# vghuy17ck1/svt-av1-psyex

Measured on AMD Instinct MI355X. Metric: ME+RD-cost Mpixels/s (2160p10 preset-6), higher is better.
Workload: dtype u8 SAD / i32 transforms; 1 GPU; 3840x2160 10-bit synthetic pan sequence, preset 6 (M6) search controls at qp 35; step = 16 pictures (4 current pictures x ref distance 1,2,4,8; R=2): open-loop ME of all 2040 b64 + full-pel pred + RD chain (64x64,32x32,16x16 DCT_DCT, 10-bit, b quantizer; qcoeff + recon + scalars written); 3 picture sets alternate from step to step

## Files before the change

### include/svt_hip_dsp.h

```cpp
#ifndef SVT_HIP_DSP_H
#define SVT_HIP_DSP_H

#include <stdint.h>
#include "svt_hip_me.h"

#ifdef __cplusplus
extern "C" {
#endif

#define SVT_HIP_TX_SIZES_ALL 19
#define SVT_HIP_TX_TYPES 16

typedef struct SvtHipQuantRow {
    int16_t zbin[2], round[2], quant[2], quant_shift[2];
    int16_t round_fp[2], quant_fp[2];
    int16_t dequant[2];
} SvtHipQuantRow;

typedef struct SvtHipTxJob {
    uint32_t src_offset;
    uint32_t pred_offset;
    uint8_t  tx_type;
    uint8_t  quant_row;
    uint8_t  pf_shape;
// ... 27 lines not shown
typedef struct SvtHipFwdTxBatchDesc {
    uint8_t  tx_size, reserved[3];
    uint32_t n_jobs;
    uint32_t residual_stride;
    const int16_t     *residual;
    const SvtHipTxJob *jobs;
    int32_t           *coeff;
} SvtHipFwdTxBatchDesc;
int svt_hip_fwd_txfm_batch(SvtHipContext *ctx, const SvtHipFwdTxBatchDesc *d);

typedef struct SvtHipInvTxBatchDesc {
    uint8_t  bit_depth;
    uint8_t  sample_bytes;
    uint8_t  tx_size;
    uint8_t  reserved;
    uint32_t n_jobs;
    uint32_t pred_stride, recon_stride;
    const void        *pred;
    void              *recon;
    const SvtHipTxJob *jobs;
    const int32_t     *dqcoeff;
} SvtHipInvTxBatchDesc;
int svt_hip_inv_txfm_batch(SvtHipContext *ctx, const SvtHipInvTxBatchDesc *d);

typedef struct SvtHipBlockJob {
    uint32_t src_offset, ref_offset;
    uint8_t  width, height;
    uint8_t  subpel_x, subpel_y;
} SvtHipBlockJob;

typedef struct SvtHipBlockStatsDesc {
    uint8_t  bit_depth;
    uint8_t  temporal_layer_index;
    uint8_t  spy_rd;
    uint8_t  reserved;
    uint32_t n_jobs;
    uint32_t src_stride, ref_stride;
    const void           *src, *ref;
    const SvtHipBlockJob *jobs;
    uint32_t *sad;
    uint64_t *sse;
    uint32_t *variance;
    uint32_t *var_sse;
    uint32_t *satd;
    double    psy_rd;
    uint64_t *psy_energy;
// ... 157 lines not shown
```

### svt-av1-psyex_amd/api.py

```python
import ctypes as C
import os

import numpy as np

from . import abi

_HERE = os.path.dirname(os.path.abspath(__file__))
LIB_PATH = os.environ.get("SVT_HIP_LIBRARY") or os.path.join(_HERE, "libsvthip.so")
_lib = None

ERRORS = {1: "no usable gfx950 device", 2: "bad parameter", 3: "out of device memory", 4: "launch/stream error"}


class SvtHipError(RuntimeError):
    pass


def lib():
    global _lib
    if _lib is None:
        if not os.path.exists(LIB_PATH):
            raise SvtHipError(f"{LIB_PATH} is missing: build it with `make -C svt-av1-psyex_amd/csrc` "
                              "(or __graft_entry__.build()); there is no CPU fallback")
        try:
# ... 127 lines not shown
        self.check(lib().svt_hip_context_set_me_counting(self._h, 1 if on else 0), "svt_hip_context_set_me_counting")

    def me_dense_counters(self):
        v = (C.c_ulonglong * 2)()
        self.check(lib().svt_hip_me_dense_counters(self._h, v), "svt_hip_me_dense_counters")
        return int(v[0]), int(v[1])

    ME_DENSE_PATHS = ("fast", "partial_row", "skip_line", "short", "odd", "octet", "off")

    def set_me_dense_fast(self, on):
        self.check(lib().svt_hip_context_set_me_dense_fast(self._h, 1 if on else 0), "svt_hip_context_set_me_dense_fast")

    def set_me_dense_plan(self, plan):
        self.check(lib().svt_hip_context_set_me_dense_plan(self._h, int(plan)), "svt_hip_context_set_me_dense_plan")

    def me_dense_path_counters(self):
        n = len(self.ME_DENSE_PATHS)
        v = (C.c_ulonglong * (2 * n + 7))()
        self.check(lib().svt_hip_me_dense_path_counters(self._h, v), "svt_hip_me_dense_path_counters")
        out = {name: (int(v[2 * i]), int(v[2 * i + 1])) for i, name in enumerate(self.ME_DENSE_PATHS)}
        out["fast_rows"] = {8 * (m + 2): int(v[2 * n + m]) for m in range(7)}
        return out

    def me_dense_slots(self):
        L = lib()
        n = C.c_size_t()
        L.svt_hip_me_dense_slots.argtypes = [C.c_void_p, C.c_void_p, C.c_size_t, C.POINTER(C.c_size_t)]
        self.check(L.svt_hip_me_dense_slots(self._h, None, 0, C.byref(n)), "svt_hip_me_dense_slots")
        out = np.zeros(n.value // 16, dtype=[("key", "<u8"), ("org", "<u4"), ("size", "<u4")])
        self.check(L.svt_hip_me_dense_slots(self._h, out.ctypes.data_as(C.c_void_p), out.nbytes, C.byref(n)), "svt_hip_me_dense_slots")
        return out

    def upload(self, host_pyramid, device_pyramid=True):
        pic = C.c_void_p()
        full = host_pyramid.desc(2)
        if device_pyramid:
            rc = lib().svt_hip_pa_picture_create(self._h, C.byref(full), None, None, C.byref(pic))
        else:
            q, s = host_pyramid.desc(1), host_pyramid.desc(0)
            rc = lib().svt_hip_pa_picture_create(self._h, C.byref(full), C.byref(q), C.byref(s), C.byref(pic))
        self.check(rc, "svt_hip_pa_picture_create")
        return DevicePicture(self, pic, host_pyramid.picture_number)

    def upload_dev(self, dev_ptr, stride, width, height, pad, picture_number=0):
        pic = C.c_void_p()
        full = abi.PlaneDesc(dev_ptr, stride, pad, pad, width, height)
# ... 78 lines not shown
```

### svt-av1-psyex_amd/csrc/rd_kernel.hip

```cpp
#include <hip/hip_runtime.h>
#include <math.h>
#include <stdint.h>
#include <string.h>
#include <type_traits>
#include "svt_hip_internal.h"
#include "batch_host.h"
#include "../../include/svt_hip_dsp.h"

#include "txfm_core.h"

namespace {

struct RdParams {
    SvtHipRdBatchDesc d;
    const int16_t    *iscan[3];
    int               tx_size;
};

template <typename T> __device__ __forceinline__ int ldpix(const void *p, size_t i) { return (int)static_cast<const T *>(p)[i]; }

__host__ __device__ constexpr int rd_lanes_per_block(int ts) { return tx_wide(ts) > tx_high(ts) ? tx_wide(ts) : tx_high(ts); }
__host__ __device__ constexpr int rd_blocks_per_wave(int ts) { return 64 / rd_lanes_per_block(ts); }

#ifndef SVT_RD_WAVES_64
#define SVT_RD_WAVES_64 2
#endif
#ifndef SVT_RD_WAVES_32
#define SVT_RD_WAVES_32 4
#endif
#ifndef SVT_RD_RESIDUAL_AHEAD
#define SVT_RD_RESIDUAL_AHEAD 8
#endif
#ifndef SVT_RD_SCAN_AHEAD
#define SVT_RD_SCAN_AHEAD 16
#endif
#ifndef SVT_RD_WAVES_16
#define SVT_RD_WAVES_16 4
#endif
#ifndef SVT_RD_FOLD_INV_32LANE
#define SVT_RD_FOLD_INV_32LANE 1
#endif
__host__ __device__ constexpr int rd_bounded_btf(int ts) {
    return ((rd_lanes_per_block(ts) == 32 && tx_wide(ts) != tx_high(ts)) || (tx_wide(ts) == 64 && tx_high(ts) == 16)) ? 3 : 2;
}
#ifndef SVT_RD_CLAMP_FREE
#define SVT_RD_CLAMP_FREE 1
#endif
#ifndef SVT_RD_SKIP_ENTRY_CLAMPS
#define SVT_RD_SKIP_ENTRY_CLAMPS 1
#endif
#ifndef SVT_RD_PAIR_RESIDUAL_MAX
#define SVT_RD_PAIR_RESIDUAL_MAX 1
#endif
#ifndef SVT_RD_ROW_BOUND_FROM_QUANT
#define SVT_RD_ROW_BOUND_FROM_QUANT 1
#endif
__host__ __device__ constexpr bool rd_clamp_free_tier(int ts) {
    return tx_wide(ts) == tx_high(ts) && (SVT_RD_CLAMP_FREE == 1 ? tx_wide(ts) == 64 : SVT_RD_CLAMP_FREE == 2 && tx_wide(ts) >= 16);
}
__host__ __device__ constexpr bool rd_skip_entry_clamps(int ts) { return SVT_RD_SKIP_ENTRY_CLAMPS && rd_bounded_btf(ts) == 2; }
#ifdef SVT_RD_TIER_STATS
__device__ unsigned int g_rd_tier_stats[10];
#endif
template <bool FREE> __device__ __forceinline__ int ipass_tier(uint32_t wave_max_abs_input, int n, int clamp_bits) {
    if (FREE && ipass_clamp_free(wave_max_abs_input, n, clamp_bits)) return 2;
    return ipass_fits_18_bits(wave_max_abs_input, n) ? 1 : 0;
}
__host__ __device__ constexpr int rd_waves_per_simd(int ts) {
    return rd_lanes_per_block(ts) == 64 ? SVT_RD_WAVES_64 : rd_lanes_per_block(ts) == 32 ? SVT_RD_WAVES_32 : SVT_RD_WAVES_16;
}
template <int TS, int BD> __global__ void __launch_bounds__(64, rd_waves_per_simd(TS)) rd_tx_kernel(const RdParams p) {
    constexpr int W = tx_wide(TS), H = tx_high(TS), WP = W > 32 ? 32 : W, HP = H > 32 ? 32 : H, NP = WP * HP;
    constexpr int LW = rd_lanes_per_block(TS), BPW = rd_blocks_per_wave(TS);
    constexpr bool kShift32 = LW != 32;
    constexpr bool kFoldInv = LW != 32 || SVT_RD_FOLD_INV_32LANE;
    constexpr int kBtf = rd_bounded_btf(TS);
    constexpr bool kFree = rd_clamp_free_tier(TS), kSkipEntry = rd_skip_entry_clamps(TS);
    constexpr int PA = W + 1, PB = WP + 1;
    constexpr int ROW_CLAMP = BD == 8 ? 16 : 18, COL_CLAMP = 16;
    constexpr bool RECT = (W == 2 * H || H == 2 * W);
    using Pix = typename std::conditional<BD == 8, uint8_t, uint16_t>::type;
    __shared__ int32_t lds[BPW][H * PA];
    const int      lane = threadIdx.x, blk = lane / LW, l = lane % LW;
    const uint32_t job   = blockIdx.x * BPW + blk;
    const bool     valid = job < p.d.n_jobs;
    int32_t *A = lds[blk];
    const SvtHipTxJob jb = p.d.jobs[valid ? job : 0];
    const int tt = jb.tx_type & 15, vt = c_vtx[tt], ht = c_htx[tt];
    const bool ud = (vt == 2), lr = (ht == 2);
    const Pix *src  = static_cast<const Pix *>(p.d.src) + jb.src_offset;
    const Pix *pred = static_cast<const Pix *>(p.d.pred) + jb.pred_offset;
    const int8_t *fsh = c_fwd_shift[TS];
    const int bit_col = c_fwd_cos_col[ilog2c(W) - 2][ilog2c(H) - 2], bit_row = c_fwd_cos_row[ilog2c(W) - 2][ilog2c(H) - 2];

    constexpr int RUN = W < 8 ? W : 8, RPR = W / RUN;
    typedef Pix __attribute__((ext_vector_type(RUN), aligned(sizeof(Pix)))) RunU;
    uint32_t rmax = 0;
    {
        HiLo rhl;
        constexpr int NIT = (RPR * H + LW - 1) / LW, kResidualAhead = NIT < SVT_RD_RESIDUAL_AHEAD ? NIT : SVT_RD_RESIDUAL_AHEAD;
        for (int it0 = 0; it0 < NIT; it0 += kResidualAhead) {
            RunU sv[kResidualAhead], pv[kResidualAhead];
#pragma unroll
            for (int j = 0; j < kResidualAhead; j++) {
                const int i = l + (it0 + j) * LW;
                if (it0 + j < NIT && i < RPR * H) {
                    const int r = i / RPR, c = (i - r * RPR) * RUN;
                    sv[j] = *reinterpret_cast<const RunU *>(src + (size_t)r * p.d.src_stride + c);
                    pv[j] = *reinterpret_cast<const RunU *>(pred + (size_t)r * p.d.pred_stride + c);
                }
            }
#pragma unroll
// ... 2 lines not shown
                if (it0 + j < NIT && i < RPR * H) {
                    const int r = i / RPR, c = (i - r * RPR) * RUN;
                    static_assert(RUN % 2 == 0, "the extremes are taken per pair of samples");
#pragma unroll
                    for (int k = 0; k < RUN; k += 2) {
                        const int32_t d0 = (int16_t)((int16_t)sv[j][k] - (int16_t)pv[j][k]), d1 = (int16_t)((int16_t)sv[j][k + 1] - (int16_t)pv[j][k + 1]);
                        A[r * PA + c + k]     = d0;
                        A[r * PA + c + k + 1] = d1;
#if SVT_RD_PAIR_RESIDUAL_MAX
                        rhl.take(d0, d1);
#else
                        rhl.take(d0);
                        rhl.take(d1);
#endif
                    }
                }
            }
        }
        rmax = rhl.max_abs();
    }
    const bool fast_col = pass_fits_17_bits((uint32_t)__builtin_amdgcn_readfirstlane((int)wave_max(rmax)) << (fsh[0] > 0 ? fsh[0] : 0), H);
    __syncthreads();
    uint32_t cmax = 0;
    if (l < W) {
        int32_t x[H];
#pragma unroll
        for (int r = 0; r < H; r++) x[r] = A[(ud ? H - 1 - r : r) * PA + l];
        shift_vec<H>(x, fsh[0]);
        if constexpr (kBtf == 2) {
#pragma unroll
            for (int r = 0; r < H; r++) x[r] = held_in_vgpr(x[r]);
        }
        if (fast_col) fwd_1d_bounded<H, kShift32, kBtf>(x, vt, bit_col, fsh[1]); else { fwd_1d<H, 0>(x, vt, bit_col); shift_vec<H>(x, fsh[1]); }
        const int oc = lr ? W - 1 - l : l;
#pragma unroll
        for (int r = 0; r < H; r++) A[r * PA + oc] = x[r];
        cmax = vec_max_abs<H>(x);
    }
    const bool fast_row = pass_fits_17_bits((uint32_t)__builtin_amdgcn_readfirstlane((int)wave_max(cmax)), W);
    __syncthreads();
    uint32_t comax = 0;
    if (l < H) {
        int32_t x[W];
#pragma unroll
        for (int c = 0; c < W; c++) x[c] = A[l * PA + c];
        if (fast_row) fwd_1d_bounded<W, kShift32, kBtf>(x, ht, bit_row, fsh[2]); else { fwd_1d<W, 0>(x, ht, bit_row); shift_vec<W>(x, fsh[2]); }
        if constexpr (RECT) {
#pragma unroll
            for (int c = 0; c < W; c++) x[c] = rshift64((i64)x[c] * 5793, 12);
        }
#pragma unroll
        for (int c = 0; c < W; c++) A[l * PA + c] = x[c];
        comax = vec_max_abs<W>(x);
    }
    const uint32_t comax_w = (uint32_t)__builtin_amdgcn_readfirstlane((int)wave_max(comax));
    const bool q24 = comax_w < (1u << 16);
    __syncthreads();
    const int pf = jb.pf_shape & 3;
    const int keep_w = pf == 3 ? 1 : (W >> pf), keep_h = pf == 3 ? 1 : (H >> pf);
    u64 tq = 0;
    if (pf == 0) if constexpr (W > 32 || H > 32) {
        for (int i = l; i < W * H; i += LW) {
            const int r = i / W, c = i - r * W;
            if (r >= HP || c >= WP) { const int32_t v = A[r * PA + c]; tq += (u64)((i64)v * v); }
        }
// ... 6 lines not shown
    const uint8_t *qm = (tt < 9) ? p.d.qmatrix : nullptr, *iqm = (tt < 9) ? p.d.iqmatrix : nullptr;
    uint32_t satd = 0, eob = 0, qsum = 0;
    int32_t  dc_q = 0;
    u64      dres = 0, dpred = 0;
    int32_t *co_out = (p.d.coeff && valid) ? p.d.coeff + (size_t)job * NP : nullptr;
    int32_t *q_out  = (p.d.qcoeff && valid) ? p.d.qcoeff + (size_t)job * NP : nullptr;
    int32_t *dq_out = (p.d.dqcoeff && valid) ? p.d.dqcoeff + (size_t)job * NP : nullptr;
    const int32_t zb_c[2]  = {log_scale ? ((q.zbin[0] + (1 << (log_scale - 1))) >> log_scale) : q.zbin[0], log_scale ? ((q.zbin[1] + (1 << (log_scale - 1))) >> log_scale) : q.zbin[1]};
    const int32_t rnd_c[2] = {log_scale ? ((q.round[0] + (1 << (log_scale - 1))) >> log_scale) : q.round[0], log_scale ? ((q.round[1] + (1 << (log_scale - 1))) >> log_scale) : q.round[1]};
    const bool fast_q = q24 && !qm && p.d.quant_kind == 0 && !co_out && !dq_out && __all(pf == 0);
    constexpr int LS = tx_log_scale(TS), KT = LS == 2 ? 4 : 3;
    bool lane_lean = fast_q && q_out != nullptr && log_scale == LS;
    bool lane_row_free = false;
    {
        const int32_t  rndm = rnd_c[0] > rnd_c[1] ? rnd_c[0] : rnd_c[1], sm = q.quant_shift[0] > q.quant_shift[1] ? q.quant_shift[0] : q.quant_shift[1];
        const int32_t  dm = q.dequant[0] > q.dequant[1] ? q.dequant[0] : q.dequant[1], qm2 = (q.quant[0] > q.quant[1] ? q.quant[0] : q.quant[1]) + 65536;
        const bool     nonneg = (rnd_c[0] | rnd_c[1] | q.quant_shift[0] | q.quant_shift[1] | q.dequant[0] | q.dequant[1]) >= 0;
        uint32_t       tmax = comax_w + (uint32_t)(nonneg ? rndm : 0);
        if (BD == 8) tmax = tmax > 32767u ? 32767u : tmax;
        const u64 qvmax = ((((u64)tmax * (uint32_t)qm2) >> 11) * (u64)(uint32_t)(nonneg ? sm : 0)) >> (21 - LS);
        const u64 dqmax = (qvmax * (u64)(uint32_t)(nonneg ? dm : 0)) >> LS;
        const u64 M = dqmax > comax_w ? dqmax : (u64)comax_w;
        lane_lean = lane_lean && nonneg && tmax < (1u << (18 - KT)) && M < (1u << 16) && M * M * (NP / LW) < (1ull << 32);
        if constexpr (kFree && SVT_RD_ROW_BOUND_FROM_QUANT)
            lane_row_free = lane_lean && ipass_clamp_free((uint32_t)(RECT ? (M * 2896 + 2048) >> 12 : M), W, ROW_CLAMP);
    }
    const bool lean_q = __all(lane_lean);
    const bool row_free_q = kFree && SVT_RD_ROW_BOUND_FROM_QUANT && __all(lane_row_free);
    if (lean_q) {
        static_assert(NP % LW == 0, "every lane of a block walks the same number of coefficients");
        constexpr int kScanAhead = NP / LW < SVT_RD_SCAN_AHEAD ? ((NP / LW) & ~1) : SVT_RD_SCAN_AHEAD;
        static_assert(kScanAhead >= 2 && kScanAhead % 2 == 0 && NP / LW >= kScanAhead, "ahead of the loop");
        uint32_t scan2[kScanAhead / 2];
#pragma unroll
        for (int k = 0; k < kScanAhead; k += 2) scan2[k / 2] = (uint32_t)(uint16_t)iscan[l + LW * k] | ((uint32_t)(uint16_t)iscan[l + LW * (k + 1)] << 16);
        uint32_t dres32 = 0, dpred32 = 0;
        int32_t  last = -1;
        auto one = [&](int rc, int32_t zbr, int32_t rnd, uint32_t qq, uint32_t qshift, int32_t deq, int ahead = -1) {
            const int r = rc / WP, c = rc - r * WP;
            const int32_t co = A[r * PA + c], sg = (co >> 31) | 1, tu = __mul24(co, sg) + rnd;
            satd += (uint32_t)tu;
            uint32_t t = (uint32_t)tu;
            if (BD == 8) t = t > 32767u ? 32767u : t;
            const uint32_t tmp = umul24_lo(t, qq) >> 11;
            uint32_t qv = umul24_hi(tmp << KT, qshift);
            qv = tu >= zbr ? qv : 0u;
            const int32_t qs = __mul24((int32_t)qv, sg);
            int32_t dqs;
            if constexpr (LS == 0) dqs = __mul24(qs, deq);
            else dqs = __mul24(__mul24((int32_t)qv, deq) >> LS, sg);
            const int32_t dd = co - dqs;
// ... 146 lines not shown
        A[r * PB + c] = dqs;
        if (co_out) co_out[rc] = co;
        if (q_out) q_out[rc] = qs;
        if (dq_out) dq_out[rc] = dqs;
    }
    satd  = group_sum<LW>(satd);
    qsum  = group_sum<LW>(qsum);
    eob   = group_max<LW>(eob);
    dres  = group_sum<LW>(dres);
    dpred = group_sum<LW>(dpred);
    __syncthreads();
    int32_t xr[W];
    uint32_t irmax = 0;
    if (l < H) {
#pragma unroll
        for (int c = 0; c < W; c++) {
            int32_t v = (l < HP && c < WP) ? A[l * PB + c] : 0;
            if constexpr (RECT) v = rshift64((i64)v * 2896, 12);
            xr[c] = kSkipEntry ? v : clampv(v, BD + 8);
        }
        if (!row_free_q) irmax = vec_max_abs<W>(xr);
    }
    const uint32_t irmax_w = (uint32_t)__builtin_amdgcn_readfirstlane((int)wave_max(irmax));
    const int irow_tier = row_free_q ? 2 : ipass_tier<kFree>(irmax_w, W, ROW_CLAMP);
    uint32_t icmax = 0;
    if (l < H) {
        if (kSkipEntry && irmax_w >= (1u << (BD + 7))) {
#pragma unroll
            for (int c = 0; c < W; c++) xr[c] = clampv(xr[c], BD + 8);
        }
        if (irow_tier == 2) inv_1d_bounded<W, -1, kShift32, kFoldInv, kBtf>(xr, ht, c_inv_shift0[TS]);
        else if (irow_tier == 1) inv_1d_bounded<W, ROW_CLAMP, kShift32, kFoldInv, kBtf>(xr, ht, c_inv_shift0[TS]);
        else { inv_1d<W, ROW_CLAMP, 1>(xr, ht); shift_vec<W, kShift32>(xr, c_inv_shift0[TS]); }
#pragma unroll
        for (int c = 0; c < W; c++) A[l * PA + c] = xr[c];
        icmax = vec_max_abs<W>(xr);
    }
    const uint32_t icmax_w = (uint32_t)__builtin_amdgcn_readfirstlane((int)wave_max(icmax));
    const int icol_tier = ipass_tier<kFree>(icmax_w, H, COL_CLAMP);
#ifdef SVT_RD_TIER_STATS
    if (lane == 0) { atomicAdd(&g_rd_tier_stats[irow_tier * 3 + icol_tier], 1u); if (row_free_q) atomicAdd(&g_rd_tier_stats[9], 1u); }
#endif
    __syncthreads();
    u64 sse = 0;
    if (l < W) {
        int32_t x[H];
        const int ic = lr ? W - 1 - l : l;
        constexpr int kColIn = BD + 6 > 16 ? BD + 6 : 16;
#pragma unroll
        for (int r = 0; r < H; r++) x[r] = (r < HP) ? (kSkipEntry ? A[r * PA + ic] : clampv(A[r * PA + ic], kColIn)) : 0;
        if (kSkipEntry && icmax_w >= (1u << (kColIn - 1))) {
#pragma unroll
            for (int r = 0; r < HP; r++) x[r] = clampv(x[r], kColIn);
        }
        if (icol_tier == 2) inv_1d_bounded<H, -1, kShift32, kFoldInv, kBtf>(x, vt, -4);
        else if (icol_tier == 1) inv_1d_bounded<H, COL_CLAMP, kShift32, kFoldInv, kBtf>(x, vt, -4);
        else { inv_1d<H, COL_CLAMP, 1>(x, vt); shift_vec<H, kShift32>(x, -4); }
#pragma unroll
        for (int r = 0; r < H; r++) A[r * PA + l] = x[ud ? H - 1 - r : r];
    }
    __syncthreads();
    {
        Pix *rec = (p.d.recon && valid) ? static_cast<Pix *>(p.d.recon) + jb.pred_offset : nullptr;
        constexpr int NIT = (RPR * H + LW - 1) / LW;
        RunU pv[NIT], sv[NIT];
#pragma unroll
        for (int it = 0; it < NIT; it++) {
            const int i = l + it * LW;
            if (i < RPR * H) {
                const int r = i / RPR, c = (i - r * RPR) * RUN;
                pv[it] = *reinterpret_cast<const RunU *>(pred + (size_t)r * p.d.pred_stride + c);
                sv[it] = *reinterpret_cast<const RunU *>(src + (size_t)r * p.d.src_stride + c);
            }
        }
#pragma unroll
        for (int it = 0; it < NIT; it++) {
            const int i = l + it * LW;
            if (i < RPR * H) {
                const int r = i / RPR, c = (i - r * RPR) * RUN;
                RunU out;
#pragma unroll
                for (int k = 0; k < RUN; k++) {
                    int v = (int)pv[it][k] + A[r * PA + c + k];
                    v = v < 0 ? 0 : (v > (1 << BD) - 1 ? (1 << BD) - 1 : v);
                    out[k] = (Pix)v;
                    const int e = (int)sv[it][k] - v;
                    sse += (u64)((uint32_t)e * (uint32_t)e);
                }
                if (rec) *reinterpret_cast<RunU *>(rec + (size_t)r * p.d.pred_stride + c) = out;
            }
        }
    }
    sse = group_sum<LW>(sse);
    if (l == 0 && valid) {
        p.d.eob[job]  = (uint16_t)eob;
        p.d.satd[job] = satd;
        p.d.dist_coeff[2 * (size_t)job]     = dres;
        p.d.dist_coeff[2 * (size_t)job + 1] = dpred;
        p.d.three_quad_energy[job] = tq;
        p.d.sse[job]  = sse;
        if (p.d.cul_level) p.d.cul_level[job] = (uint8_t)((qsum > 63 ? 63 : qsum) | (dc_q < 0 ? 64 : 0)) + (uint8_t)(dc_q > 0 ? 128 : 0);
    }
}

struct InvParams {
    SvtHipInvTxBatchDesc d;
};
template <int TS, int BD, typename Pix> __global__ void __launch_bounds__(64, rd_waves_per_simd(TS)) inv_tx_kernel(const InvParams p) {
    constexpr int W = tx_wide(TS), H = tx_high(TS), WP = W > 32 ? 32 : W, HP = H > 32 ? 32 : H, NP = WP * HP;
    constexpr int LW = rd_lanes_per_block(TS), BPW = rd_blocks_per_wave(TS);
    constexpr bool kShift32 = LW != 32, kFoldInv = LW != 32 || SVT_RD_FOLD_INV_32LANE;
    constexpr int kBtf = rd_bounded_btf(TS);
    constexpr bool kFree = rd_clamp_free_tier(TS), kSkipEntry = rd_skip_entry_clamps(TS);
    constexpr int PA = W + 1, PB = WP + 1;
    constexpr int ROW_CLAMP = BD == 8 ? 16 : 18, COL_CLAMP = 16;
    constexpr bool RECT = (W == 2 * H || H == 2 * W);
    __shared__ int32_t lds[BPW][H * PA];
    const int      lane = threadIdx.x, blk = lane / LW, l = lane % LW;
    const uint32_t job   = blockIdx.x * BPW + blk;
    const bool     valid = job < p.d.n_jobs;
    int32_t *A = lds[blk];
    const SvtHipTxJob jb = p.d.jobs[valid ? job : 0];
    const int tt = jb.tx_type & 15, vt = c_vtx[tt], ht = c_htx[tt];
    const bool ud = (vt == 2), lr = (ht == 2);
    const Pix *pred = static_cast<const Pix *>(p.d.pred) + jb.pred_offset;
    const int32_t *dq = p.d.dqcoeff + (size_t)(valid ? job : 0) * NP;
    for (int rc = l; rc < NP; rc += LW) { const int r = rc / WP, c = rc - r * WP; A[r * PB + c] = dq[rc]; }
    __syncthreads();
    int32_t xr[W];
    uint32_t irmax = 0;
    if (l < H) {
#pragma unroll
        for (int c = 0; c < W; c++) {
            int32_t v = (l < HP && c < WP) ? A[l * PB + c] : 0;
            if constexpr (RECT) v = rshift64((i64)v * 2896, 12);
            xr[c] = kSkipEntry ? v : clampv(v, BD + 8);
        }
        irmax = vec_max_abs<W>(xr);
    }
    const uint32_t irmax_w = (uint32_t)__builtin_amdgcn_readfirstlane((int)wave_max(irmax));
    const int irow_tier = ipass_tier<kFree>(irmax_w, W, ROW_CLAMP);
    uint32_t icmax = 0;
    if (l < H) {
        if (kSkipEntry && irmax_w >= (1u << (BD + 7))) {
#pragma unroll
            for (int c = 0; c < W; c++) xr[c] = clampv(xr[c], BD + 8);
        }
        if (irow_tier == 2) inv_1d_bounded<W, -1, kShift32, kFoldInv, kBtf>(xr, ht, c_inv_shift0[TS]);
        else if (irow_tier == 1) inv_1d_bounded<W, ROW_CLAMP, kShift32, kFoldInv, kBtf>(xr, ht, c_inv_shift0[TS]);
        else { inv_1d<W, ROW_CLAMP, 1>(xr, ht); shift_vec<W, kShift32>(xr, c_inv_shift0[TS]); }
#pragma unroll
        for (int c = 0; c < W; c++) A[l * PA + c] = xr[c];
        icmax = vec_max_abs<W>(xr);
    }
    const uint32_t icmax_w = (uint32_t)__builtin_amdgcn_readfirstlane((int)wave_max(icmax));
    const int icol_tier = ipass_tier<kFree>(icmax_w, H, COL_CLAMP);
    __syncthreads();
    if (l < W) {
        int32_t x[H];
        const int ic = lr ? W - 1 - l : l;
        constexpr int kColIn = BD + 6 > 16 ? BD + 6 : 16;
#pragma unroll
        for (int r = 0; r < H; r++) x[r] = (r < HP) ? (kSkipEntry ? A[r * PA + ic] : clampv(A[r * PA + ic], kColIn)) : 0;
        if (kSkipEntry && icmax_w >= (1u << (kColIn - 1))) {
#pragma unroll
            for (int r = 0; r < HP; r++) x[r] = clampv(x[r], kColIn);
        }
        if (icol_tier == 2) inv_1d_bounded<H, -1, kShift32, kFoldInv, kBtf>(x, vt, -4);
        else if (icol_tier == 1) inv_1d_bounded<H, COL_CLAMP, kShift32, kFoldInv, kBtf>(x, vt, -4);
        else { inv_1d<H, COL_CLAMP, 1>(x, vt); shift_vec<H, kShift32>(x, -4); }
#pragma unroll
        for (int r = 0; r < H; r++) A[r * PA + l] = x[ud ? H - 1 - r : r];
    }
    __syncthreads();
    if (valid) {
        Pix *rec = static_cast<Pix *>(p.d.recon) + jb.src_offset;
        for (int i = l; i < W * H; i += LW) {
            const int r = i / W, c = i - r * W;
            int v = (int)pred[(size_t)r * p.d.pred_stride + c] + A[r * PA + c];
            v = v < 0 ? 0 : (v > (1 << BD) - 1 ? (1 << BD) - 1 : v);
            rec[(size_t)r * p.d.recon_stride + c] = (Pix)v;
        }
    }
}

template <int BD, typename Pix> void launch_inv(SvtHipContext *ctx, const InvParams &p) {
    const dim3 b(64);
#define CASE(S) case S: hipLaunchKernelGGL((inv_tx_kernel<S, BD, Pix>), dim3(ceil_div(p.d.n_jobs, rd_blocks_per_wave(S))), b, 0, ctx->stream, p); break;
    switch (p.d.tx_size) {
        CASE(0) CASE(1) CASE(2) CASE(3) CASE(4) CASE(5) CASE(6) CASE(7) CASE(8) CASE(9) CASE(10) CASE(11) CASE(12) CASE(13) CASE(14) CASE(15) CASE(16) CASE(17) CASE(18)
    }
#undef CASE
}

struct FwdParams {
// ... 96 lines not shown

extern "C" {

int svt_hip_tx_size_wide(int tx_size) { return (tx_size >= 0 && tx_size < 19) ? tx_wide(tx_size) : 0; }
int svt_hip_tx_size_high(int tx_size) { return (tx_size >= 0 && tx_size < 19) ? tx_high(tx_size) : 0; }

int svt_hip_scan_order(int tx_size, int tx_type, int16_t *scan, int16_t *iscan) {
    if (tx_size < 0 || tx_size >= 19 || tx_type < 0 || tx_type >= 16 || !scan || !iscan) return 0;
    return scan_order(tx_size, tx_type, scan, iscan);
}

static int rd_batch_check(const SvtHipRdBatchDesc *d) {
    if (d->n_jobs == 0) return SVT_HIP_OK;
    if ((d->bit_depth != 8 && d->bit_depth != 10) || d->quant_kind > 2) BAD("bit_depth %u / quant_kind %u", d->bit_depth, d->quant_kind);
    if (!d->src || !d->pred || !d->jobs || !d->quant_rows || !d->eob || !d->satd || !d->dist_coeff || !d->three_quad_energy || !d->sse)
        BAD("a mandatory pointer of the RD batch is null");
    if ((d->qmatrix == nullptr) != (d->iqmatrix == nullptr)) BAD("qmatrix and iqmatrix go together");
    if (d->tx_size >= SVT_HIP_TX_SIZES_ALL) BAD("tx_size %d", d->tx_size);
    return SVT_HIP_OK;
}

int svt_hip_rd_batch(SvtHipContext *ctx, const SvtHipRdBatchDesc *d) {
    const int rc = enqueue_batch("svt_hip_rd_batch", ctx, d, rd_batch_check, &SvtHipRdBatchDesc::n_jobs, [=] {
        RdParams p = {*d, {}, d->tx_size};
        for (int k = 0; k < 3; k++) p.iscan[k] = ctx->iscan_dev + ((size_t)p.tx_size * 3 + k) * 1024;
        if (d->bit_depth == 8) launch_size<8>(ctx, p);
        else launch_size<10>(ctx, p);
    });
#ifdef SVT_RD_TIER_STATS
    unsigned int st[10] = {0}, zero[10] = {0};
    if (rc == SVT_HIP_OK && d->n_jobs && hipStreamSynchronize(ctx->stream) == hipSuccess &&
        hipMemcpyFromSymbol(st, HIP_SYMBOL(g_rd_tier_stats), sizeof(st)) == hipSuccess && hipMemcpyToSymbol(HIP_SYMBOL(g_rd_tier_stats), zero, sizeof(zero)) == hipSuccess)
        fprintf(stderr, "rd_tier_stats tx_size %d jobs %u  row x col (0 general, 1 bounded, 2 clamp-free): %u %u %u | %u %u %u | %u %u %u  row tier from the quantizer: %u\n",
                d->tx_size, d->n_jobs, st[0], st[1], st[2], st[3], st[4], st[5], st[6], st[7], st[8], st[9]);
#endif
    return rc;
}

}

namespace {
template <typename Pix> __device__ __forceinline__ void fullpel_pred_b64(const Pix *ref, uint32_t ref_stride, int width, int height, const uint32_t *sb_best_mv,
                                                                         int list, int ref_idx, uint32_t w64, int bx, int by, Pix *pred, uint32_t pred_stride,
                                                                         int vec_ok) {
    typedef Pix __attribute__((ext_vector_type(8), aligned(sizeof(Pix)))) RunU;
    typedef Pix __attribute__((ext_vector_type(8))) Run;
    const uint32_t b = (uint32_t)bx + (uint32_t)by * w64;
    const uint32_t *mvs = sb_best_mv + ((size_t)b * 8 + list * 4 + ref_idx) * 85 + 5;
    for (int seg = threadIdx.x; seg < 64 * 8; seg += 256) {
        const int ly = seg >> 3, lx = (seg & 7) * 8, x = bx * 64 + lx, y = by * 64 + ly;
        if (x >= width || y >= height) continue;
        const int qx = lx >> 4, qy = ly >> 4;
        const uint32_t mv = mvs[(qx & 1) | ((qy & 1) << 1) | ((qx >> 1) << 2) | ((qy >> 1) << 3)];
        const int mvx = (int16_t)(mv & 0xFFFF), mvy = (int16_t)(mv >> 16);
        int sy = y + mvy;
        sy = sy < 0 ? 0 : (sy > height - 1 ? height - 1 : sy);
        const int sx = x + mvx;
        const Pix *srow = ref + (size_t)sy * ref_stride;
        Pix       *drow = pred + (size_t)y * pred_stride + x;
// ... 67 lines not shown
        if (j.b64_row_count == 0 || j.b64_row_start + j.b64_row_count > h64) j.b64_row_count = h64 - j.b64_row_start;
        rows_max = j.b64_row_count > rows_max ? j.b64_row_count : rows_max;
        vec_ok   = vec_ok && (reinterpret_cast<uintptr_t>(j.pred) % (8 * bpp)) == 0;
        pb.job[i] = j;
    }
    const dim3 g(w64, rows_max, n_jobs), blk(256);
    return enqueue_locked("svt_hip_fullpel_pred_batch", ctx, [&] {
        if (bit_depth == 8) hipLaunchKernelGGL(fullpel_pred_batch_kernel<uint8_t>, g, blk, 0, ctx->stream, pb, ref_stride, (int)width, (int)height, w64, pred_stride, vec_ok);
        else hipLaunchKernelGGL(fullpel_pred_batch_kernel<uint16_t>, g, blk, 0, ctx->stream, pb, ref_stride, (int)width, (int)height, w64, pred_stride, vec_ok);
    });
}

static int inv_txfm_check(const SvtHipInvTxBatchDesc *d) {
    if (d->n_jobs == 0) return SVT_HIP_OK;
    if ((d->bit_depth != 8 && d->bit_depth != 10) || (d->sample_bytes != 1 && d->sample_bytes != 2) || (d->bit_depth == 10 && d->sample_bytes != 2))
        BAD("inverse batch: bit_depth %u with %u-byte samples", d->bit_depth, d->sample_bytes);
    if (d->tx_size >= SVT_HIP_TX_SIZES_ALL) BAD("tx_size %u", d->tx_size);
    if (!d->pred || !d->recon || !d->jobs || !d->dqcoeff) BAD("a pointer of the inverse batch is null");
    return SVT_HIP_OK;
}

extern "C" int svt_hip_inv_txfm_batch(SvtHipContext *ctx, const SvtHipInvTxBatchDesc *d) {
    return enqueue_batch("svt_hip_inv_txfm_batch", ctx, d, inv_txfm_check, &SvtHipInvTxBatchDesc::n_jobs, [=] {
        const InvParams p = {*d};
        if (d->bit_depth == 10) launch_inv<10, uint16_t>(ctx, p);
        else if (d->sample_bytes == 1) launch_inv<8, uint8_t>(ctx, p);
        else launch_inv<8, uint16_t>(ctx, p);
    });
}

static int fwd_txfm_check(const SvtHipFwdTxBatchDesc *d) {
    if (d->n_jobs == 0) return SVT_HIP_OK;
    if (d->tx_size >= SVT_HIP_TX_SIZES_ALL) BAD("tx_size %u", d->tx_size);
    if (!d->residual || !d->jobs || !d->coeff) BAD("a pointer of the forward batch is null");
    return SVT_HIP_OK;
}

extern "C" int svt_hip_fwd_txfm_batch(SvtHipContext *ctx, const SvtHipFwdTxBatchDesc *d) {
    return enqueue_batch("svt_hip_fwd_txfm_batch", ctx, d, fwd_txfm_check, &SvtHipFwdTxBatchDesc::n_jobs, [=] { launch_fwd(ctx, FwdParams{*d}); });
}

int svt_hip_rd_tables_init(SvtHipContext *ctx) {
    SVT_HIP_CHECK(ctx, txfm_upload_cospi());
    const size_t bytes = sizeof(int16_t) * 19 * 3 * 1024;
    int16_t *tab = static_cast<int16_t *>(calloc(1, bytes)), scan[1024];
    if (!tab) return svt_hip_fail(ctx, SVT_HIP_ERR_NO_MEMORY, "iscan tables");
    for (int s = 0; s < 19; s++)
        for (int kind = 0; kind < 3; kind++) scan_order(s, kind == 0 ? 0 : (kind == 1 ? 10 : 11), scan, tab + ((size_t)s * 3 + kind) * 1024);
    int rc = SVT_HIP_OK;
    if (hipMalloc(reinterpret_cast<void **>(&ctx->iscan_dev), bytes) != hipSuccess) rc = svt_hip_fail(ctx, SVT_HIP_ERR_NO_MEMORY, "iscan tables");
    else if (hipMemcpy(ctx->iscan_dev, tab, bytes, hipMemcpyHostToDevice) != hipSuccess) rc = svt_hip_fail(ctx, SVT_HIP_ERR_LAUNCH, "iscan tables: copy failed");
    free(tab);
    return rc;
}

void svt_hip_rd_tables_free(SvtHipContext *ctx) {
    if (ctx->iscan_dev) hipFree(ctx->iscan_dev);
    ctx->iscan_dev = nullptr;
}
```

### svt-av1-psyex_amd/csrc/svt_hip_internal.h

```cpp
#ifndef SVT_HIP_INTERNAL_H
#define SVT_HIP_INTERNAL_H
#include <hip/hip_runtime_api.h>
#include <stdarg.h>
#include <stdio.h>
#include <condition_variable>
#include <mutex>
#include "me_kernel.h"

#define SVT_HIP_LANES 9
#define SVT_HIP_PARAM_RING 4

struct SvtHipLane {
    hipStream_t stream;
    uint32_t   *queue_head;
    uint8_t    *params_dev;
    uint8_t    *params_host[SVT_HIP_PARAM_RING];
    hipEvent_t  params_copied[SVT_HIP_PARAM_RING];
    int         ring_next;
    void       *scratch;
    size_t      scratch_bytes;
    void       *dense;
    size_t      dense_bytes;
    size_t      dense_used;
    unsigned long long dense_seq;
// ... 12 lines not shown
    std::mutex  async_mu;
    std::mutex  pool_mu;
    std::condition_variable pool_cv;
    uint32_t    lane_busy;
    int16_t    *iscan_dev;
    bool        me_attr_set;
    int         me_staged;
    bool        me_counting;
    bool        me_timing;
    bool        me_dense;
    uint32_t    me_waves_per_cu;
    hipStream_t io_stream;
    hipEvent_t  io_fence;
    void       *tpl_scratch;
    size_t      tpl_scratch_bytes;
    void       *tpl_group_dev;
    void       *tpl_group_host;
    hipEvent_t  tpl_group_done[4];
    int         tpl_group_next;
    bool        me_dense_fast;
    int         me_dense_plan;
    unsigned long long me_dense_seq;
    uint32_t    me_max_waves;
    uint32_t    lvmap_max_grid;
};

struct SvtHipPaPicture {
    DevPyramid  pyr;
    void       *mem[3];
    size_t      bytes[3];
    hipEvent_t  ready;
    hipStream_t ready_stream;
};

char *svt_hip_err_buf(void);
#define SVT_HIP_ERR_BYTES 512

static inline int svt_hip_fail(SvtHipContext *, int code, const char *fmt, ...) {
    va_list ap;
    va_start(ap, fmt);
    vsnprintf(svt_hip_err_buf(), SVT_HIP_ERR_BYTES, fmt, ap);
    va_end(ap);
    return code;
}

#define SVT_HIP_CHECK(ctx, call)                                                                                  \
// ... 35 lines not shown
```

Before: 47650 Mpixels/s.

## Add DCT-only specialized transform passes for square 16/64 RD waves

When every lane in a wave has tx_type DCT_DCT, square transforms (16x16 and 64x64 by default mask) take specialised forward and inverse passes that skip flip indexing and type dispatch. Such waves can also use the clamp-free tier, including 16x16 through the quantizer-derived row bound. The change also swaps the compile-time tier stats for optional runtime path counters, which add a null-pointer check and a rare atomic. The specialised paths add code size and register pressure, and a wave with mixed types still takes the generic path.

Result: no change. 48110 Mpixels/s (median of 6 runs) (+1.0%).

```diff
diff --git a/include/svt_hip_dsp.h b/include/svt_hip_dsp.h
--- a/include/svt_hip_dsp.h
+++ b/include/svt_hip_dsp.h
@@ -73,6 +73,10 @@
     const int32_t     *dqcoeff;
 } SvtHipInvTxBatchDesc;
 int svt_hip_inv_txfm_batch(SvtHipContext *ctx, const SvtHipInvTxBatchDesc *d);
+
+#define SVT_HIP_RD_PATH_COUNTERS 19
+int svt_hip_context_set_rd_counting(SvtHipContext *ctx, int on);
+int svt_hip_rd_path_counters(SvtHipContext *ctx, unsigned long long out[SVT_HIP_RD_PATH_COUNTERS]);
 
 typedef struct SvtHipBlockJob {
     uint32_t src_offset, ref_offset;
diff --git a/svt-av1-psyex_amd/api.py b/svt-av1-psyex_amd/api.py
--- a/svt-av1-psyex_amd/api.py
+++ b/svt-av1-psyex_amd/api.py
@@ -173,6 +173,16 @@
         out["fast_rows"] = {8 * (m + 2): int(v[2 * n + m]) for m in range(7)}
         return out
 
+    def set_rd_counting(self, on):
+        self.check(lib().svt_hip_context_set_rd_counting(self._h, 1 if on else 0), "svt_hip_context_set_rd_counting")
+
+    def rd_path_counters(self):
+        v = (C.c_ulonglong * 19)()
+        self.check(lib().svt_hip_rd_path_counters(self._h, v), "svt_hip_rd_path_counters")
+        out = {(path, r, c): int(v[9 * p + 3 * r + c]) for p, path in enumerate(("generic", "dct")) for r in range(3) for c in range(3) if v[9 * p + 3 * r + c]}
+        out["row_from_quant"] = int(v[18])
+        return out
+
     def me_dense_slots(self):
         L = lib()
         n = C.c_size_t()
diff --git a/svt-av1-psyex_amd/csrc/rd_kernel.hip b/svt-av1-psyex_amd/csrc/rd_kernel.hip
--- a/svt-av1-psyex_amd/csrc/rd_kernel.hip
+++ b/svt-av1-psyex_amd/csrc/rd_kernel.hip
@@ -15,6 +15,7 @@
     SvtHipRdBatchDesc d;
     const int16_t    *iscan[3];
     int               tx_size;
+    unsigned int     *counters;
 };
 
 template <typename T> __device__ __forceinline__ int ldpix(const void *p, size_t i) { return (int)static_cast<const T *>(p)[i]; }
@@ -59,15 +60,87 @@
     return tx_wide(ts) == tx_high(ts) && (SVT_RD_CLAMP_FREE == 1 ? tx_wide(ts) == 64 : SVT_RD_CLAMP_FREE == 2 && tx_wide(ts) >= 16);
 }
 __host__ __device__ constexpr bool rd_skip_entry_clamps(int ts) { return SVT_RD_SKIP_ENTRY_CLAMPS && rd_bounded_btf(ts) == 2; }
-#ifdef SVT_RD_TIER_STATS
-__device__ unsigned int g_rd_tier_stats[10];
-#endif
+#ifndef SVT_RD_DCT_PATH
+#define SVT_RD_DCT_PATH 5
+#endif
+#ifndef SVT_RD_DCT_FREE
+#define SVT_RD_DCT_FREE 1
+#endif
+__host__ __device__ constexpr bool rd_dct_path(int ts) { return tx_wide(ts) == tx_high(ts) && tx_wide(ts) >= 16 && ((SVT_RD_DCT_PATH >> (ilog2c(tx_wide(ts)) - 4)) & 1); }
+__host__ __device__ constexpr bool rd_dct_free_tier(int ts) {
+    return rd_dct_path(ts) && (rd_clamp_free_tier(ts) || (tx_wide(ts) == 16 && (SVT_RD_DCT_FREE & 1)) || (tx_wide(ts) == 32 && (SVT_RD_DCT_FREE & 2)));
+}
 template <bool FREE> __device__ __forceinline__ int ipass_tier(uint32_t wave_max_abs_input, int n, int clamp_bits) {
     if (FREE && ipass_clamp_free(wave_max_abs_input, n, clamp_bits)) return 2;
     return ipass_fits_18_bits(wave_max_abs_input, n) ? 1 : 0;
 }
 __host__ __device__ constexpr int rd_waves_per_simd(int ts) {
     return rd_lanes_per_block(ts) == 64 ? SVT_RD_WAVES_64 : rd_lanes_per_block(ts) == 32 ? SVT_RD_WAVES_32 : SVT_RD_WAVES_16;
+}
+template <int TS> struct RdDctGeom {
+    static constexpr int N = tx_wide(TS), NP = N > 32 ? 32 : N, PA = N + 1, PB = NP + 1;
+    static constexpr bool kShift32 = rd_lanes_per_block(TS) != 32, kFoldInv = rd_lanes_per_block(TS) != 32 || SVT_RD_FOLD_INV_32LANE;
+    static_assert(!rd_dct_path(TS) || (tx_wide(TS) == tx_high(TS) && rd_bounded_btf(TS) == 2 && rd_skip_entry_clamps(TS)), "what the passes below assume");
+};
+template <int TS> __device__ __forceinline__ uint32_t rd_dct_fwd_cols(int32_t *A, int l, bool fast_col, int bit_col, const int8_t *fsh) {
+    using G = RdDctGeom<TS>;
+    constexpr int N = G::N, PA = G::PA;
+    int32_t x[N];
+#pragma unroll
+    for (int r = 0; r < N; r++) x[r] = A[r * PA + l];
+    shift_vec<N>(x, fsh[0]);
+    if (fast_col) fwd_1d_bounded<N, G::kShift32, 2>(x, 0, bit_col, fsh[1]); else { fwd_1d<N, 0>(x, 0, bit_col); shift_vec<N>(x, fsh[1]); }
+#pragma unroll
+    for (int r = 0; r < N; r++) A[r * PA + l] = x[r];
+    return vec_max_abs<N>(x);
+}
+template <int TS> __device__ __forceinline__ uint32_t rd_dct_fwd_rows(int32_t *A, int l, bool fast_row, int bit_row, int sh) {
+    using G = RdDctGeom<TS>;
+    constexpr int N = G::N, PA = G::PA;
+    int32_t x[N];
+#pragma unroll
+    for (int c = 0; c < N; c++) x[c] = A[l * PA + c];
+    if (fast_row) fwd_1d_bounded<N, G::kShift32, 2>(x, 0, bit_row, sh); else { fwd_1d<N, 0>(x, 0, bit_row); shift_vec<N>(x, sh); }
+#pragma unroll
+    for (int c = 0; c < N; c++) A[l * PA + c] = x[c];
+    return vec_max_abs<N>(x);
+}
+template <int TS, int BD> __device__ __forceinline__ uint32_t rd_dct_inv_rows(int32_t *xr, int32_t *A, int l, int tier, uint32_t irmax_w) {
+    using G = RdDctGeom<TS>;
+    constexpr int N = G::N, PA = G::PA, ROW_CLAMP = BD == 8 ? 16 : 18;
+    if (tier == 2) inv_1d_bounded<N, -1, G::kShift32, G::kFoldInv, 2>(xr, 0, c_inv_shift0[TS]);
+    else {
+        if (irmax_w >= (1u << (BD + 7))) {
+#pragma unroll
+            for (int c = 0; c < N; c++) xr[c] = clampv(xr[c], BD + 8);
+        }
+        if (tier == 1) inv_1d_bounded<N, ROW_CLAMP, G::kShift32, G::kFoldInv, 2>(xr, 0, c_inv_shift0[TS]);
+        else { inv_1d<N, ROW_CLAMP, 1>(xr, 0); shift_vec<N, G::kShift32>(xr, c_inv_shift0[TS]); }
+    }
+#pragma unroll
+    for (int c = 0; c < N; c++) A[l * PA + c] = xr[c];
+    return vec_max_abs<N>(xr);
+}
+template <int TS, int BD> __device__ __forceinline__ void rd_dct_inv_cols(int32_t *A, int l, int tier, uint32_t icmax_w) {
+    using G = RdDctGeom<TS>;
+    constexpr int N = G::N, NP = G::NP, PA = G::PA, COL_CLAMP = 16, kColIn = BD + 6 > 16 ? BD + 6 : 16;
+    int32_t x[N];
+#pragma unroll
+    for (int r = 0; r < N; r++) x[r] = (r < NP) ? A[r * PA + l] : 0;
+    if (tier == 2) inv_1d_bounded<N, -1, G::kShift32, G::kFoldInv, 2>(x, 0, -4);
+    else {
+        if (icmax_w >= (1u << (kColIn - 1))) {
+#pragma unroll
+            for (int r = 0; r < NP; r++) x[r] = clampv(x[r], kColIn);
+        }
+        if (tier == 1) inv_1d_bounded<N, COL_CLAMP, G::kShift32, G::kFoldInv, 2>(x, 0, -4);
+        else { inv_1d<N, COL_CLAMP, 1>(x, 0); shift_vec<N, G::kShift32>(x, -4); }
+    }
+#pragma unroll
+    for (int r = 0; r < N; r++) A[r * PA + l] = x[r];
+}
+__device__ __forceinline__ void rd_count_wave(unsigned int *counters, int lane, bool dct_wave, int irow_tier, int icol_tier, bool row_from_quant) {
+    if (counters && lane < 2 && (lane == 0 || row_from_quant)) atomicAdd(counters + (lane ? 18 : (dct_wave ? 9 : 0) + 3 * irow_tier + icol_tier), 1u);
 }
 template <int TS, int BD> __global__ void __launch_bounds__(64, rd_waves_per_simd(TS)) rd_tx_kernel(const RdParams p) {
     constexpr int W = tx_wide(TS), H = tx_high(TS), WP = W > 32 ? 32 : W, HP = H > 32 ? 32 : H, NP = WP * HP;
@@ -76,6 +149,7 @@
     constexpr bool kFoldInv = LW != 32 || SVT_RD_FOLD_INV_32LANE;
     constexpr int kBtf = rd_bounded_btf(TS);
     constexpr bool kFree = rd_clamp_free_tier(TS), kSkipEntry = rd_skip_entry_clamps(TS);
+    constexpr bool kDct = rd_dct_path(TS), kFreeDct = rd_dct_free_tier(TS);
     constexpr int PA = W + 1, PB = WP + 1;
     constexpr int ROW_CLAMP = BD == 8 ? 16 : 18, COL_CLAMP = 16;
     constexpr bool RECT = (W == 2 * H || H == 2 * W);
@@ -88,6 +162,7 @@
     const SvtHipTxJob jb = p.d.jobs[valid ? job : 0];
     const int tt = jb.tx_type & 15, vt = c_vtx[tt], ht = c_htx[tt];
     const bool ud = (vt == 2), lr = (ht == 2);
+    const bool dct_wave = kDct && __all(tt == 0);
     const Pix *src  = static_cast<const Pix *>(p.d.src) + jb.src_offset;
     const Pix *pred = static_cast<const Pix *>(p.d.pred) + jb.pred_offset;
     const int8_t *fsh = c_fwd_shift[TS];
@@ -136,7 +211,8 @@
     const bool fast_col = pass_fits_17_bits((uint32_t)__builtin_amdgcn_readfirstlane((int)wave_max(rmax)) << (fsh[0] > 0 ? fsh[0] : 0), H);
     __syncthreads();
     uint32_t cmax = 0;
-    if (l < W) {
+    if (dct_wave) cmax = rd_dct_fwd_cols<TS>(A, l, fast_col, bit_col, fsh);
+    else if (l < W) {
         int32_t x[H];
 #pragma unroll
         for (int r = 0; r < H; r++) x[r] = A[(ud ? H - 1 - r : r) * PA + l];
@@ -154,7 +230,8 @@
     const bool fast_row = pass_fits_17_bits((uint32_t)__builtin_amdgcn_readfirstlane((int)wave_max(cmax)), W);
     __syncthreads();
     uint32_t comax = 0;
-    if (l < H) {
+    if (dct_wave) comax = rd_dct_fwd_rows<TS>(A, l, fast_row, bit_row, fsh[2]);
+    else if (l < H) {
         int32_t x[W];
 #pragma unroll
         for (int c = 0; c < W; c++) x[c] = A[l * PA + c];
@@ -207,11 +284,11 @@
         const u64 dqmax = (qvmax * (u64)(uint32_t)(nonneg ? dm : 0)) >> LS;
         const u64 M = dqmax > comax_w ? dqmax : (u64)comax_w;
         lane_lean = lane_lean && nonneg && tmax < (1u << (18 - KT)) && M < (1u << 16) && M * M * (NP / LW) < (1ull << 32);
-        if constexpr (kFree && SVT_RD_ROW_BOUND_FROM_QUANT)
+        if constexpr ((kFree || kFreeDct) && SVT_RD_ROW_BOUND_FROM_QUANT)
             lane_row_free = lane_lean && ipass_clamp_free((uint32_t)(RECT ? (M * 2896 + 2048) >> 12 : M), W, ROW_CLAMP);
     }
     const bool lean_q = __all(lane_lean);
-    const bool row_free_q = kFree && SVT_RD_ROW_BOUND_FROM_QUANT && __all(lane_row_free);
+    const bool row_free_q = (dct_wave ? kFreeDct : kFree) && SVT_RD_ROW_BOUND_FROM_QUANT && __all(lane_row_free);
     if (lean_q) {
         static_assert(NP % LW == 0, "every lane of a block walks the same number of coefficients");
         constexpr int kScanAhead = NP / LW < SVT_RD_SCAN_AHEAD ? ((NP / LW) & ~1) : SVT_RD_SCAN_AHEAD;
@@ -404,9 +481,10 @@
         if (!row_free_q) irmax = vec_max_abs<W>(xr);
     }
     const uint32_t irmax_w = (uint32_t)__builtin_amdgcn_readfirstlane((int)wave_max(irmax));
-    const int irow_tier = row_free_q ? 2 : ipass_tier<kFree>(irmax_w, W, ROW_CLAMP);
+    const int irow_tier = row_free_q ? 2 : (dct_wave ? ipass_tier<kFreeDct>(irmax_w, W, ROW_CLAMP) : ipass_tier<kFree>(irmax_w, W, ROW_CLAMP));
     uint32_t icmax = 0;
-    if (l < H) {
+    if (dct_wave) icmax = rd_dct_inv_rows<TS, BD>(xr, A, l, irow_tier, irmax_w);
+    else if (l < H) {
         if (kSkipEntry && irmax_w >= (1u << (BD + 7))) {
 #pragma unroll
             for (int c = 0; c < W; c++) xr[c] = clampv(xr[c], BD + 8);
@@ -419,13 +497,11 @@
         icmax = vec_max_abs<W>(xr);
     }
     const uint32_t icmax_w = (uint32_t)__builtin_amdgcn_readfirstlane((int)wave_max(icmax));
-    const int icol_tier = ipass_tier<kFree>(icmax_w, H, COL_CLAMP);
-#ifdef SVT_RD_TIER_STATS
-    if (lane == 0) { atomicAdd(&g_rd_tier_stats[irow_tier * 3 + icol_tier], 1u); if (row_free_q) atomicAdd(&g_rd_tier_stats[9], 1u); }
-#endif
+    const int icol_tier = dct_wave ? ipass_tier<kFreeDct>(icmax_w, H, COL_CLAMP) : ipass_tier<kFree>(icmax_w, H, COL_CLAMP);
     __syncthreads();
     u64 sse = 0;
-    if (l < W) {
+    if (dct_wave) rd_dct_inv_cols<TS, BD>(A, l, icol_tier, icmax_w);
+    else if (l < W) {
         int32_t x[H];
         const int ic = lr ? W - 1 - l : l;
         constexpr int kColIn = BD + 6 > 16 ? BD + 6 : 16;
@@ -439,7 +515,7 @@
         else if (icol_tier == 1) inv_1d_bounded<H, COL_CLAMP, kShift32, kFoldInv, kBtf>(x, vt, -4);
         else { inv_1d<H, COL_CLAMP, 1>(x, vt); shift_vec<H, kShift32>(x, -4); }
 #pragma unroll
-        for (int r = 0; r < H; r++) A[r * PA + l] = x[ud ? H - 1 - r : r];
+        for (int r = 0; r < H; r++) A[r * PA + l] = ud ? x[H - 1 - r] : x[r];
     }
     __syncthreads();
     {
@@ -474,6 +550,7 @@
         }
     }
     sse = group_sum<LW>(sse);
+    if constexpr (kDct) rd_count_wave(p.counters, lane, dct_wave, irow_tier, icol_tier, row_free_q);
     if (l == 0 && valid) {
         p.d.eob[job]  = (uint16_t)eob;
         p.d.satd[job] = satd;
@@ -487,6 +564,7 @@
 
 struct InvParams {
     SvtHipInvTxBatchDesc d;
+    unsigned int        *counters;
 };
 template <int TS, int BD, typename Pix> __global__ void __launch_bounds__(64, rd_waves_per_simd(TS)) inv_tx_kernel(const InvParams p) {
     constexpr int W = tx_wide(TS), H = tx_high(TS), WP = W > 32 ? 32 : W, HP = H > 32 ? 32 : H, NP = WP * HP;
@@ -494,6 +572,7 @@
     constexpr bool kShift32 = LW != 32, kFoldInv = LW != 32 || SVT_RD_FOLD_INV_32LANE;
     constexpr int kBtf = rd_bounded_btf(TS);
     constexpr bool kFree = rd_clamp_free_tier(TS), kSkipEntry = rd_skip_entry_clamps(TS);
+    constexpr bool kDct = rd_dct_path(TS), kFreeDct = rd_dct_free_tier(TS);
     constexpr int PA = W + 1, PB = WP + 1;
     constexpr int ROW_CLAMP = BD == 8 ? 16 : 18, COL_CLAMP = 16;
     constexpr bool RECT = (W == 2 * H || H == 2 * W);
@@ -505,6 +584,7 @@
     const SvtHipTxJob jb = p.d.jobs[valid ? job : 0];
     const int tt = jb.tx_type & 15, vt = c_vtx[tt], ht = c_htx[tt];
     const bool ud = (vt == 2), lr = (ht == 2);
+    const bool dct_wave = kDct && __all(tt == 0);
     const Pix *pred = static_cast<const Pix *>(p.d.pred) + jb.pred_offset;
     const int32_t *dq = p.d.dqcoeff + (size_t)(valid ? job : 0) * NP;
     for (int rc = l; rc < NP; rc += LW) { const int r = rc / WP, c = rc - r * WP; A[r * PB + c] = dq[rc]; }
@@ -521,9 +601,10 @@
         irmax = vec_max_abs<W>(xr);
     }
     const uint32_t irmax_w = (uint32_t)__builtin_amdgcn_readfirstlane((int)wave_max(irmax));
-    const int irow_tier = ipass_tier<kFree>(irmax_w, W, ROW_CLAMP);
+    const int irow_tier = dct_wave ? ipass_tier<kFreeDct>(irmax_w, W, ROW_CLAMP) : ipass_tier<kFree>(irmax_w, W, ROW_CLAMP);
     uint32_t icmax = 0;
-    if (l < H) {
+    if (dct_wave) icmax = rd_dct_inv_rows<TS, BD>(xr, A, l, irow_tier, irmax_w);
+    else if (l < H) {
         if (kSkipEntry && irmax_w >= (1u << (BD + 7))) {
 #pragma unroll
             for (int c = 0; c < W; c++) xr[c] = clampv(xr[c], BD + 8);
@@ -536,9 +617,11 @@
         icmax = vec_max_abs<W>(xr);
     }
     const uint32_t icmax_w = (uint32_t)__builtin_amdgcn_readfirstlane((int)wave_max(icmax));
-    const int icol_tier = ipass_tier<kFree>(icmax_w, H, COL_CLAMP);
-    __syncthreads();
-    if (l < W) {
+    const int icol_tier = dct_wave ? ipass_tier<kFreeDct>(icmax_w, H, COL_CLAMP) : ipass_tier<kFree>(icmax_w, H, COL_CLAMP);
+    if constexpr (kDct) rd_count_wave(p.counters, lane, dct_wave, irow_tier, icol_tier, false);
+    __syncthreads();
+    if (dct_wave) rd_dct_inv_cols<TS, BD>(A, l, icol_tier, icmax_w);
+    else if (l < W) {
         int32_t x[H];
         const int ic = lr ? W - 1 - l : l;
         constexpr int kColIn = BD + 6 > 16 ? BD + 6 : 16;
@@ -552,7 +635,7 @@
         else if (icol_tier == 1) inv_1d_bounded<H, COL_CLAMP, kShift32, kFoldInv, kBtf>(x, vt, -4);
         else { inv_1d<H, COL_CLAMP, 1>(x, vt); shift_vec<H, kShift32>(x, -4); }
 #pragma unroll
-        for (int r = 0; r < H; r++) A[r * PA + l] = x[ud ? H - 1 - r : r];
+        for (int r = 0; r < H; r++) A[r * PA + l] = ud ? x[H - 1 - r] : x[r];
     }
     __syncthreads();
     if (valid) {
@@ -695,19 +778,31 @@
 
 int svt_hip_rd_batch(SvtHipContext *ctx, const SvtHipRdBatchDesc *d) {
     const int rc = enqueue_batch("svt_hip_rd_batch", ctx, d, rd_batch_check, &SvtHipRdBatchDesc::n_jobs, [=] {
-        RdParams p = {*d, {}, d->tx_size};
+        RdParams p = {*d, {}, d->tx_size, ctx->rd_counting ? ctx->rd_counters_dev : nullptr};
         for (int k = 0; k < 3; k++) p.iscan[k] = ctx->iscan_dev + ((size_t)p.tx_size * 3 + k) * 1024;
         if (d->bit_depth == 8) launch_size<8>(ctx, p);
         else launch_size<10>(ctx, p);
     });
-#ifdef SVT_RD_TIER_STATS
-    unsigned int st[10] = {0}, zero[10] = {0};
-    if (rc == SVT_HIP_OK && d->n_jobs && hipStreamSynchronize(ctx->stream) == hipSuccess &&
-        hipMemcpyFromSymbol(st, HIP_SYMBOL(g_rd_tier_stats), sizeof(st)) == hipSuccess && hipMemcpyToSymbol(HIP_SYMBOL(g_rd_tier_stats), zero, sizeof(zero)) == hipSuccess)
-        fprintf(stderr, "rd_tier_stats tx_size %d jobs %u  row x col (0 general, 1 bounded, 2 clamp-free): %u %u %u | %u %u %u | %u %u %u  row tier from the quantizer: %u\n",
-                d->tx_size, d->n_jobs, st[0], st[1], st[2], st[3], st[4], st[5], st[6], st[7], st[8], st[9]);
-#endif
     return rc;
+}
+
+int svt_hip_context_set_rd_counting(SvtHipContext *ctx, int on) {
+    if (!ctx) return SVT_HIP_ERR_BAD_PARAM;
+    ctx->rd_counting = on != 0;
+    return SVT_HIP_OK;
+}
+
+int svt_hip_rd_path_counters(SvtHipContext *ctx, unsigned long long out[SVT_HIP_RD_PATH_COUNTERS]) {
+    if (!ctx || !out) return SVT_HIP_ERR_BAD_PARAM;
+    unsigned int v[SVT_HIP_RD_PATH_COUNTERS];
+    hipSetDevice(ctx->device);
+    for (int i = 0; i < SVT_HIP_LANES; i++) {
+        if (ctx->lane[i].ready) SVT_HIP_CHECK(ctx, hipStreamSynchronize(ctx->lane[i].stream));
+    }
+    SVT_HIP_CHECK(ctx, hipMemcpy(v, ctx->rd_counters_dev, sizeof(v), hipMemcpyDeviceToHost));
+    SVT_HIP_CHECK(ctx, hipMemset(ctx->rd_counters_dev, 0, sizeof(v)));
+    for (int k = 0; k < SVT_HIP_RD_PATH_COUNTERS; k++) out[k] = v[k];
+    return SVT_HIP_OK;
 }
 
 }
@@ -821,7 +916,7 @@
 
 extern "C" int svt_hip_inv_txfm_batch(SvtHipContext *ctx, const SvtHipInvTxBatchDesc *d) {
     return enqueue_batch("svt_hip_inv_txfm_batch", ctx, d, inv_txfm_check, &SvtHipInvTxBatchDesc::n_jobs, [=] {
-        const InvParams p = {*d};
+        const InvParams p = {*d, ctx->rd_counting ? ctx->rd_counters_dev : nullptr};
         if (d->bit_depth == 10) launch_inv<10, uint16_t>(ctx, p);
         else if (d->sample_bytes == 1) launch_inv<8, uint8_t>(ctx, p);
         else launch_inv<8, uint16_t>(ctx, p);
@@ -850,10 +945,16 @@
     if (hipMalloc(reinterpret_cast<void **>(&ctx->iscan_dev), bytes) != hipSuccess) rc = svt_hip_fail(ctx, SVT_HIP_ERR_NO_MEMORY, "iscan tables");
     else if (hipMemcpy(ctx->iscan_dev, tab, bytes, hipMemcpyHostToDevice) != hipSuccess) rc = svt_hip_fail(ctx, SVT_HIP_ERR_LAUNCH, "iscan tables: copy failed");
     free(tab);
+    if (rc != SVT_HIP_OK) return rc;
+    if (hipMalloc(reinterpret_cast<void **>(&ctx->rd_counters_dev), SVT_HIP_RD_PATH_COUNTERS * sizeof(unsigned int)) != hipSuccess)
+        return svt_hip_fail(ctx, SVT_HIP_ERR_NO_MEMORY, "RD path counters");
+    SVT_HIP_CHECK(ctx, hipMemset(ctx->rd_counters_dev, 0, SVT_HIP_RD_PATH_COUNTERS * sizeof(unsigned int)));
     return rc;
 }
 
 void svt_hip_rd_tables_free(SvtHipContext *ctx) {
     if (ctx->iscan_dev) hipFree(ctx->iscan_dev);
+    if (ctx->rd_counters_dev) hipFree(ctx->rd_counters_dev);
     ctx->iscan_dev = nullptr;
-}
+    ctx->rd_counters_dev = nullptr;
+}
diff --git a/svt-av1-psyex_amd/csrc/svt_hip_internal.h b/svt-av1-psyex_amd/csrc/svt_hip_internal.h
--- a/svt-av1-psyex_amd/csrc/svt_hip_internal.h
+++ b/svt-av1-psyex_amd/csrc/svt_hip_internal.h
@@ -58,6 +58,8 @@
     int         me_dense_plan;
     unsigned long long me_dense_seq;
     uint32_t    me_max_waves;
+    bool        rd_counting;
+    unsigned int *rd_counters_dev;
     uint32_t    lvmap_max_grid;
 };
 
```
